# MattiaDallaCosta/JPEG-encoder-decoder

Measured on AMD Instinct MI355X. Metric: Mpixels/s encoded (device-resident BGR888 -> JFIF bytes), higher is better.
Workload: dtype int8-MFMA exact + fp64 replay (bit-exact); 1 GPU; config 3: 256 x 3840x2160 BGR888 frames per GPU, 4:2:0, Q=50, one independent JFIF per frame; frames_per_gpu=256, width=3840, height=2160, quality=50, mode=encode, pipeline=fused, parallelism=frame-parallel x1

## Files before the change

jpeg-encoder-decoder_amd/csrc/mij_kernels.hip:

```cpp
#include <stdlib.h>

#include "mij_internal.h"
#include "mij_headers.h"
#include "mij_colour_f64.h"

namespace mij {

typedef int v4i __attribute__((ext_vector_type(4)));
typedef unsigned u4v __attribute__((ext_vector_type(4)));
typedef unsigned short us2 __attribute__((ext_vector_type(2)));

__constant__ int c_zigzag[64] = {
    0,  1,  8,  16, 9,  2,  3,  10, 17, 24, 32, 25, 18, 11, 4,  5,
    12, 19, 26, 33, 40, 48, 41, 34, 27, 20, 13, 6,  7,  14, 21, 28,
    35, 42, 49, 56, 57, 50, 43, 36, 29, 22, 15, 23, 30, 37, 44, 51,
    58, 59, 52, 45, 38, 31, 39, 46, 53, 60, 61, 54, 47, 55, 62, 63};

#define SQRT1_2 0.70710678118654752440

__device__ __forceinline__ void wave_lds_sync() {
  __builtin_amdgcn_fence(__ATOMIC_RELEASE, "wavefront");
  __builtin_amdgcn_wave_barrier();
  __builtin_amdgcn_fence(__ATOMIC_ACQUIRE, "wavefront");
}

template <int N>
__device__ __forceinline__ uint32_t row_shr0(uint32_t x) {
  return (uint32_t)__builtin_amdgcn_update_dpp(0, (int)x, 0x110 + N, 0xF, 0xF, true);
}
__device__ __forceinline__ uint32_t row_scan16(uint32_t x) {
  x += row_shr0<1>(x);
  x += row_shr0<2>(x);
  x += row_shr0<4>(x);
  x += row_shr0<8>(x);
  return x;
}
__device__ __forceinline__ uint32_t row_last(uint32_t x) {
  return (uint32_t)__builtin_amdgcn_update_dpp(0, (int)x, 0x15F, 0xF, 0xF, false);
}
__device__ __forceinline__ uint32_t wave_scan64(uint32_t x) {
  x = row_scan16(x);
  x += (uint32_t)__builtin_amdgcn_update_dpp(0, (int)x, 0x142, 0xA, 0xF, false);
  x += (uint32_t)__builtin_amdgcn_update_dpp(0, (int)x, 0x143, 0xC, 0xF, false);
  return x;
}

__device__ __forceinline__ int mag_class(int v) {
  v = v < 0 ? -v : v;
  return 32 - __clz(v);
}

__device__ __forceinline__ uint32_t mag_bits(int v, int cls) {
  uint32_t id = (uint32_t)(v < 0 ? -v : v);
  if (v < 0) id = ~id;
  return id & ((1u << cls) - 1u);
}

// ... 34 lines not shown
  }
  if (ey) atomicOr(&lut[0 * LUT_WORDS + (i >> 5)], 1u << (i & 31));
  if (ecb) atomicOr(&lut[1 * LUT_WORDS + (i >> 5)], 1u << (i & 31));
  if (ecr) atomicOr(&lut[2 * LUT_WORDS + (i >> 5)], 1u << (i & 31));
}


__device__ __forceinline__ int dc_exact(int S, int q) {
  double f = __dmul_rn(__dmul_rn((double)S, SQRT1_2), SQRT1_2);
  f = __dmul_rn(f, 0.25);
  int t = (int)__ddiv_rn(f, (double)q);
  return t < -2048 ? -2048 : (t > 2047 ? 2047 : t);
}

__device__ __forceinline__ int dc_fast(int S, int q8, float inv8q, bool &tie) {
  const int s = S >> 31;
  const int a = (S ^ s) - s;
  const int k = (int)fmaf((float)a, inv8q, 2e-4f);
  tie = a != 0 && k * q8 == a;
  return (k ^ s) - s;
}

__device__ __forceinline__ int dc_tie(int d, const uint32_t *bits) {
  const int s = d >> 31;
  int k = (d ^ s) - s;
  k -= (int)((bits[k >> 5] >> (k & 31)) & 1u);
  return (k ^ s) - s;
}

struct TilePos {
  int f, tx, ty, valid_px;
};

__device__ __forceinline__ TilePos tile_pos(const Geom &G, int t) {
  TilePos p;
  p.f = (int)div_by((uint32_t)t, G.tpf_m, G.tpf_s);
  const int rem = t - p.f * G.tiles_per_frame;
  p.ty = (int)div_by((uint32_t)rem, G.tx_m, G.tx_s);
  p.tx = rem - p.ty * G.tiles_x;
  p.valid_px = min(TILE_W, G.w - p.tx * TILE_W);
  return p;
}

__device__ __forceinline__ TilePos tile_pos_r(const Geom &G, const int2 *fd, int t, bool &ok) {
  TilePos p = tile_pos(G, t);
  const FGeom fg = frame_geom(G, fd, p.f);
  p.valid_px = min(TILE_W, fg.w - p.tx * TILE_W);
  ok = p.tx < fg.tiles_x && p.ty < fg.rows;
  return p;
}

typedef __attribute__((address_space(3))) void lds_void_t;
typedef __attribute__((address_space(1))) void global_void_t;
constexpr int TILE_RAW = TILE_W * 3 * TILE_H;

constexpr int DMA_K = TILE_H / 2;
struct DmaOff {
  uint32_t v;
};
__device__ __forceinline__ DmaOff dma_offsets(int pitch, int lane) {
  const int l = lane < 48 ? lane : 0;
  return DmaOff{(uint32_t)((l / 24) * pitch + (l % 24) * 16)};
}
template <int K>
__device__ __forceinline__ void dma_one(uint32_t off, uint32_t lds, const uint8_t *src) {
  asm volatile("s_mov_b32 m0, %1\n\tglobal_load_lds_dwordx4 %0, %2 nt" : : "v"(off), "s"(lds), "s"(src)
               : "memory", "m0");
}
__device__ __forceinline__ void issue_tile_dma(const K1Args &a, const TilePos &p, int lane, uint8_t *raw,
                                               const DmaOff &off) {
  const uint64_t srcv = (uint64_t)(uintptr_t)(a.in + (long long)p.f * a.in_fs +
                                              (long long)(p.ty * TILE_H) * a.pitch + p.tx * TILE_W * 3);
  const uint32_t src_hi = (uint32_t)__builtin_amdgcn_readfirstlane((uint32_t)(srcv >> 32));
  const uint32_t src_lo = (uint32_t)__builtin_amdgcn_readfirstlane((uint32_t)srcv);
  const uint8_t *src = (const uint8_t *)(uintptr_t)(((uint64_t)src_hi << 32) | (uint64_t)src_lo);
  const uint32_t lds0 = __builtin_amdgcn_readfirstlane((uint32_t)(uintptr_t)(lds_void_t *)raw);
  const long long step = 2LL * a.pitch;
  const bool on = lane < 48 && (p.valid_px == TILE_W || (lane % 24) * 16 < p.valid_px * 3);
  if (on) {
    dma_one<0>(off.v, lds0, src);
    dma_one<1>(off.v, lds0 + 768, src + step);
    dma_one<2>(off.v, lds0 + 1536, src + 2 * step);
    dma_one<3>(off.v, lds0 + 2304, src + 3 * step);
    dma_one<4>(off.v, lds0 + 3072, src + 4 * step);
    dma_one<5>(off.v, lds0 + 3840, src + 5 * step);
    dma_one<6>(off.v, lds0 + 4608, src + 6 * step);
    dma_one<7>(off.v, lds0 + 5376, src + 7 * step);
  }
}
static_assert(DMA_K == 8 && TILE_W * 3 * 2 == 768, "issue_tile_dma: 8 instructions of 2 rows x 384 B");

__device__ __forceinline__ void dma_wait() { asm volatile("s_waitcnt vmcnt(0)" ::: "memory"); }
__device__ __forceinline__ void dma_wait_behind_stores() { asm volatile("s_waitcnt vmcnt(6)" ::: "memory"); }

template <int N>
__device__ __forceinline__ float ubyte_f32(uint32_t w) {
  float r;
  if constexpr (N == 0) asm("v_cvt_f32_ubyte0 %0, %1" : "=v"(r) : "v"(w));
  else if constexpr (N == 1) asm("v_cvt_f32_ubyte1 %0, %1" : "=v"(r) : "v"(w));
  else if constexpr (N == 2) asm("v_cvt_f32_ubyte2 %0, %1" : "=v"(r) : "v"(w));
  else asm("v_cvt_f32_ubyte3 %0, %1" : "=v"(r) : "v"(w));
  return r;
}

typedef float f2v __attribute__((ext_vector_type(2)));

__device__ __forceinline__ uint32_t pack_i16x2(int lo, int hi) {
  return __builtin_amdgcn_perm((uint32_t)hi, (uint32_t)lo, 0x05040100u);
}

__device__ __forceinline__ f2v pk_add_k(f2v a, float k) {
  f2v r;
  const unsigned long long kk = __float_as_uint(k);
  asm("v_pk_add_f32 %0, %1, %2 op_sel_hi:[1,0]" : "=v"(r) : "v"(a), "s"(kk));
  return r;
}

constexpr float CH_BIAS = 127.5f + 0x1p-16f;
constexpr float MAGIC = 12582912.0f;
constexpr uint32_t MAGIC_BITS = 0x4B400000u;
// ... 159 lines not shown
    for (int dy = 0; dy < 2; dy++)
      if (__ballot(r[dy].cy)) {
        const uint32_t corr = y_fix<RGB, GLOBAL_LUT>(w[it][dy][0], w[it][dy][1], w[it][dy][2], r[dy].yb, lut,
                                                     c4 | (pr << 5));
        if (corr) *Yd[dy] = py[dy] - corr;
      }
    if (__ballot(r[0].pd * r[1].pd == 0.0f)) {
      uint32_t cbc[2][4], crc[2][4];
#pragma unroll
      for (int dy = 0; dy < 2; dy++)
        chroma_fix<RGB, GLOBAL_LUT>(w[it][dy][0], w[it][dy][1], w[it][dy][2], lut, cbc[dy], crc[dy], c4 | (pr << 5));
      const uint32_t nb0 = cbc[0][0] + cbc[0][1] + cbc[1][0] + cbc[1][1];
      const uint32_t nb1 = cbc[0][2] + cbc[0][3] + cbc[1][2] + cbc[1][3];
      const uint32_t nr0 = crc[0][0] + crc[0][1] + crc[1][0] + crc[1][1];
      const uint32_t nr1 = crc[0][2] + crc[0][3] + crc[1][2] + crc[1][3];
      if (nb0 | nb1) *(uint16_t *)C0 = (uint16_t)chroma_pair(r[0].cbm, r[1].cbm, nb0, nb1);
      if (nr0 | nr1) *(uint16_t *)(C0 + 8 * LDS_BLK) = (uint16_t)chroma_pair(r[0].crm, r[1].crm, nr0, nr1);
    }
  }
}

constexpr uint32_t TOK_AC = 1u << 10;
constexpr uint32_t LB_NOTOK = TOK_AC | 0xFFu;
constexpr uint32_t SEG_DC_ONLY = 1u << 31;

__device__ __forceinline__ uint32_t &tok_at(uint32_t *base, uint32_t i) {
  return *(uint32_t *)((char *)base + (i << 2));
}
__device__ __forceinline__ void emit_tokens(const int (&o)[16], int lane, int g, int bcol,
                                            bool valid, bool chroma, bool dc_diffed,
                                            bool first_pred, int pred0,
                                            uint32_t *segtok, uint32_t segoff, uint32_t *tok0, uint32_t *segcnt, uint32_t *hDC,
                                            uint32_t *hAC, int16_t (*st)[16], int kflags = 0, bool acz = false, bool dc_only = false) {
  if (acz && dc_only) {
    const int dc0 = o[0];
    const int prev = (int)row_shr0<1>((uint32_t)dc0);
    const unsigned long long vb = __ballot(valid && g == 0);
    if (g == 0) {
      if ((bcol & 7) == 7) *segcnt = SEG_DC_ONLY | (uint32_t)__popcll(vb);
      if (valid && (bcol & 7) != 0) atomicAdd(&hDC[mag_class(dc0 - prev)], 1u);
    }
    if (lane == 0 && vb) atomicAdd(&hAC[0x00], (unsigned)__popcll(vb));
    return;
  }
  uint32_t Mlo = 0, Mhi = 0;
  const int zsw = 8 * (bcol & 7);
  if (!acz) {
  u4v c0, c1;
#pragma unroll
  for (int k = 0; k < 4; k++) {
    c0[k] = pack_i16x2(o[2 * k], o[2 * k + 1]);
    c1[k] = pack_i16x2(o[8 + 2 * k], o[9 + 2 * k]);
  }
  int16_t *stb = &st[0][0] + 64 * bcol;
  *(u4v *)(stb + ((16 * g) ^ zsw)) = c0;
  *(u4v *)(stb + ((16 * g + 8) ^ zsw)) = c1;
  uint32_t pm;
  asm("v_pk_min_u16 %0, %1, 1 op_sel_hi:[1,0]" : "=v"(pm) : "v"(c0[0]));
#pragma unroll
  for (int k = 1; k < 8; k++) {
    const uint32_t w = k < 4 ? c0[k] : c1[k - 4];
    uint32_t h;
    asm("v_pk_min_u16 %0, %1, 1 op_sel_hi:[1,0]" : "=v"(h) : "v"(w));
    asm("v_lshl_or_b32 %0, %1, %2, %3" : "=v"(pm) : "v"(h), "i"(2 * k), "v"(pm));
  }
  uint32_t m16 = (pm & 0x5555u) | ((pm >> 15) & 0xAAAAu);
  if (g == 0) m16 &= ~1u;
  uint32_t h = m16 << (16 * (g & 1));
  const auto r16 = __builtin_amdgcn_permlane16_swap(h, h, false, false);
  h = r16[0] | r16[1];
  const auto r32 = __builtin_amdgcn_permlane32_swap(h, h, false, false);
  Mlo = r32[0];
  Mhi = r32[1];
  }
  const int eob = !(Mhi >> 31);
  const int n = valid ? 1 + __popc(Mlo) + __popc(Mhi) + eob : 0;
  const int pos = chroma ? (bcol & 7) : bcol;
  uint32_t incl = row_scan16((uint32_t)n);
  if (chroma)
    incl -= (uint32_t)__builtin_amdgcn_update_dpp(0, (int)incl, 0x157, 0xF, 0xF, false) & (0u - (uint32_t)(bcol >> 3));
  const int base = (int)incl - n;
  const int dc0 = o[0];
  const int prev = (int)row_shr0<1>((uint32_t)dc0);
  wave_lds_sync();
  if (pos == (chroma ? 7 : 15)) {
    if (g == 0) *segcnt = incl;
    if ((uint32_t)g < ((0u - incl) & 3u)) tok_at(segtok, segoff + incl + (uint32_t)g) = LB_NOTOK;
  }
  if (g == 0) {
    if (valid) {
      if (dc_diffed || pos != 0 || first_pred) {
        const int diff = dc_diffed ? dc0 : dc0 - (pos != 0 ? prev : pred0);
        const int cls = mag_class(diff);
        const uint32_t tk = (uint32_t)cls | (mag_bits(diff, cls) << 16);
        if (pos == 0) *tok0 = tk;
        else tok_at(segtok, segoff + base) = tk;
        atomicAdd(&hDC[cls], 1u);
      }
      if (eob) tok_at(segtok, segoff + base + n - 1) = TOK_AC;
    }
  }
  {
    const unsigned long long eobs = __ballot(g == 0 && valid && eob);
    if (lane == 0 && eobs) atomicAdd(&hAC[0x00], (unsigned)__popcll(eobs));
  }
  if (!acz && valid && !(kflags & K1F_NO_ACLOOP)) {
    const int16_t *sl = &st[0][0] + 64 * bcol;
    auto token = [&](int z, int rank, int zp) {
      const int cz = sl[z ^ zsw];
      const int m = cz + (cz >> 31);
      uint32_t lead;
      asm("v_ffbh_i32 %0, %1" : "=v"(lead) : "v"(m));
      const uint32_t cls = 32u - lead;
      const uint32_t mag = __builtin_amdgcn_ubfe((uint32_t)m, 0u, cls);
      const uint32_t runp = (uint32_t)(z + zp);
      const uint32_t t = (runp << 4) + cls;
      if (!(kflags & K1F_NO_TOKSTORE)) tok_at(segtok, segoff + (uint32_t)(base + rank)) = t | (mag << 16);
      if (!(kflags & K1F_NO_HIST)) {
        atomicAdd(&hAC[t & 255u], 1u);
        if (runp >= 80u) atomicAdd(&hAC[0xF0], (runp - 64u) >> 4);
      }
    };
    const uint32_t cm = 0x11111111u << g;
    const int rank_lo = __popc(Mlo), zp_lo = 31 - __clz((int)(Mlo | 1u));
    const uint32_t M1 = Mlo | 1u;
    for (uint32_t m = Mlo & cm; m; m &= m - 1u) {
      const int z = __builtin_ctz(m);
      const uint32_t bef = __builtin_amdgcn_ubfe(M1, 0u, (uint32_t)z);
      uint32_t lz;
      asm("v_ffbh_u32 %0, %1" : "=v"(lz) : "v"(bef));
      token(z, __popc(bef), 32 + (int)lz);
    }
    const int rank_lo1 = rank_lo + 1;
    for (uint32_t m = Mhi & cm; m; m &= m - 1u) {
      const int zz = __builtin_ctz(m);
      const uint32_t bef = __builtin_amdgcn_ubfe(Mhi, 0u, (uint32_t)zz);
      uint32_t lz;
      asm("v_ffbh_u32 %0, %1" : "=v"(lz) : "v"(bef));
      token(32 + zz, rank_lo1 + __popc(bef), (int)min(lz, (uint32_t)(63 - zp_lo)));
    }
  }
  wave_lds_sync();
}

constexpr int K1M_COEF_OUT = 1;
constexpr int K1M_TOK_OUT = 2;
constexpr int K1M_COEF_IN = 4;
constexpr int K1M_RGB = 8;
constexpr int K1M_REGIONS = 16;
constexpr int K1M_AUDIT = 32;
constexpr int K1M_FLOOR = 64;
constexpr int k1_base(int mode) { return mode & ~(K1M_RGB | K1M_REGIONS | K1M_AUDIT | K1M_FLOOR); }

template <int MODE>
constexpr bool k1_wide() { return k1_base(MODE) == K1M_COEF_OUT || k1_base(MODE) == K1M_TOK_OUT; }
template <int MODE>
constexpr int k1_waves() {
  return k1_wide<MODE>() ? 12 : 4;
}

template <int MODE>
__global__ __launch_bounds__(64 * k1_waves<MODE>(), k1_wide<MODE>() ? 1 : 2) void k_mcu_dct(K1Args a) {
  constexpr bool PIX = !(MODE & K1M_COEF_IN);
  constexpr bool TOK = MODE & K1M_TOK_OUT;
  constexpr int NW = k1_waves<MODE>();
  constexpr int NT = 64 * NW;
  constexpr bool DEFER = k1_base(MODE) == K1M_COEF_OUT;
  constexpr bool RGB = MODE & K1M_RGB;
  constexpr bool REG = MODE & K1M_REGIONS;
  constexpr bool AUDIT = MODE & K1M_AUDIT;
  constexpr bool FLOOR = MODE & K1M_FLOOR;
  const int2 *const fdims = REG ? a.fdims : nullptr;
  __shared__ __attribute__((aligned(16))) uint8_t s_raw[PIX ? NW : 1][TILE_RAW];
  __shared__ __attribute__((aligned(16))) uint8_t s_tile[PIX ? NW : 1][LDS_WAVE];
  __shared__ __attribute__((aligned(16))) int4 s_A[PIX ? 12 * 64 : 1];
  __shared__ __attribute__((aligned(16))) float s_fac[2][64];
  __shared__ float s_inv8q[2];
  __shared__ uint32_t s_dctie[2][DCTIE_WORDS];
  constexpr bool LUT_LDS = PIX && !(TOK && NW >= 8);
  __shared__ uint32_t s_lut[LUT_LDS ? 3 * LUT_WORDS : 1];
  __shared__ double s_cos[64];
  __shared__ uint8_t s_zz[64];
  __shared__ int s_qint[2][64];
  __shared__ __attribute__((aligned(16))) int s_czl[PIX ? 64 : 1];
  __shared__ __attribute__((aligned(16))) int16_t s_st[TOK ? NW : 1][64][16];
  constexpr int HREP = PIX ? 1 : 4;
  __shared__ uint32_t s_hac[TOK ? 2 : 1][2][HREP][256];
  __shared__ uint32_t s_hdc[TOK ? 2 : 1][2][HREP][16];
  __shared__ int s_next;

  const Tables *__restrict__ T = a.tab;
#ifdef MIJ_K1_DIAG
  const int kflags = a.flags;
#else
  constexpr int kflags = 0;
#endif
  if (threadIdx.x < 64) {
    s_cos[threadIdx.x] = T->cosd[threadIdx.x];
    s_zz[threadIdx.x] = (uint8_t)c_zigzag[threadIdx.x];
  }
  if (TOK) {
    for (int i = threadIdx.x; i < 2 * 2 * HREP * 256; i += NT) (&s_hac[0][0][0][0])[i] = 0;
    for (int i = threadIdx.x; i < 2 * 2 * HREP * 16; i += NT) (&s_hdc[0][0][0][0])[i] = 0;
  }
  if (threadIdx.x < 128) s_qint[threadIdx.x >> 6][threadIdx.x & 63] = T->qint[threadIdx.x >> 6][threadIdx.x & 63];
  if (threadIdx.x < 2) s_inv8q[threadIdx.x] = 1.0f / (float)(8 * T->qint[threadIdx.x][0]);
  if (PIX && threadIdx.x < 64) s_czl[threadIdx.x] = T->czl[threadIdx.x];
  if (threadIdx.x < 2 * DCTIE_WORDS) (&s_dctie[0][0])[threadIdx.x] = (&T->dctie[0][0])[threadIdx.x];
  if (PIX) {
    for (int i = threadIdx.x; i < 12 * 64; i += NT) s_A[i] = T->mfma_a[i];
    if (LUT_LDS)
      for (int i = threadIdx.x; i < 3 * LUT_WORDS; i += NT) s_lut[i] = (&T->lut[0][0])[i];
  }
  const uint32_t *__restrict__ lut = LUT_LDS ? (const uint32_t *)s_lut : &T->lut[0][0];
  for (int i = threadIdx.x; i < 128; i += NT) {
    s_fac[i >> 6][i & 63] = T->qfac[i >> 6][i & 63];
  }
  if (threadIdx.x == 0) s_next = (int)blockIdx.x * a.per_wg + NW;
  if (blockIdx.x == 0)
    for (int i = threadIdx.x; i < a.nerr_zero; i += NT) a.err_zero[i] = 0;
  __syncthreads();

  const int lane = threadIdx.x & 63;
  const int wave = __builtin_amdgcn_readfirstlane(threadIdx.x >> 6);
  uint8_t *L = s_tile[PIX ? wave : 0];
  const int g = lane >> 4, bcol = lane & 15;
  const int c4 = lane & 31, pr = lane >> 5;
  const uint32_t kq = (uint32_t)T->kq[g];
  const int q_dc[2] = {T->qint[0][0], T->qint[1][0]};
  const bool cz_on = PIX && !AUDIT && T->cz_on;
  const Geom &G = a.g;
  const int bw = G.w >> 3, mw = G.w >> 4;
  const int ntiles = a.nframes * G.tiles_per_frame;
  const int t0 = (int)blockIdx.x * a.per_wg;
  const int f0 = t0 / G.tiles_per_frame;
  const int tend = min(ntiles, t0 + a.per_wg);
  int t = t0 + wave;
  auto skip_outside = [&](int &tt) {
    bool ok;
    while (tt < tend && (tile_pos_r(G, fdims, tt, ok), !ok)) {
      int v = 0;
      if (lane == 0) v = atomicAdd(&s_next, 1);
      tt = __builtin_amdgcn_readfirstlane(v);
    }
  };
  auto tpos = [&](int tt) {
    bool ok;
    return REG ? tile_pos_r(G, fdims, tt, ok) : tile_pos(G, tt);
  };
  if (REG) skip_outside(t);
#ifdef MIJ_K1_DIAG
  const unsigned long long w_t0 = __builtin_amdgcn_s_memrealtime();
  int w_ntiles = 0;
  unsigned long long ph[5] = {0, 0, 0, 0, 0}, tph = __builtin_amdgcn_s_memtime();
#define K1_PHASE(k)                                                  \
  do {                                                               \
    const unsigned long long tn_ = __builtin_amdgcn_s_memtime();     \
    ph[k] += tn_ - tph;                                              \
    tph = tn_;                                                       \
  } while (0)
#else
#define K1_PHASE(k)
#endif
  uint32_t nrep = 0;
  if (t < tend) {
    uint8_t *raw = s_raw[PIX ? wave : 0];
    TilePos p = tpos(t);
    const DmaOff doff = dma_offsets(a.pitch, lane);
    if (PIX) issue_tile_dma(a, p, lane, raw, doff);
    auto load_coefs = [&](const TilePos &pp, u4v (&dst)[PIX ? 1 : 3][2]) {
#pragma unroll
      for (int nt = 0; nt < 3; nt++) {
        bool valid;
        long long blk;
        const FGeom fg = frame_geom(G, fdims, pp.f);
        const int bwf = REG ? fg.bw : bw, mwf = REG ? fg.mw : mw;
        const int nYf = REG ? fg.nY : G.nY, nCf = REG ? fg.nC : G.nC;
        if (nt < 2) {
          const int bx = pp.tx * 16 + bcol;
          valid = bx < bwf;
          blk = (long long)(2 * pp.ty + nt) * bwf + bx;
        } else {
          const int mx = pp.tx * 8 + (bcol & 7);
          valid = mx < mwf;
          blk = nYf + (bcol >= 8 ? nCf : 0) + (long long)pp.ty * mwf + mx;
        }
        dst[PIX ? 0 : nt][0] = dst[PIX ? 0 : nt][1] = u4v{0, 0, 0, 0};
        if (valid) {
          const int16_t *src = a.coef + (long long)pp.f * G.coef_fs + blk * 64 + 16 * g;
          dst[PIX ? 0 : nt][0] = *(const u4v *)src;
          dst[PIX ? 0 : nt][1] = *(const u4v *)(src + 8);
        }
      }
    };
    u4v cnext[PIX ? 1 : 3][2];
    if (!PIX) load_coefs(p, cnext);
    bool first = true;
    for (;;) {
      TilePos pn = p;
      int tn = 0;
      if (lane == 0) tn = atomicAdd(&s_next, 1);
      tn = __builtin_amdgcn_readfirstlane(tn);
      uint32_t fl_w = 0;
      if (PIX) {
        K1_PHASE(3);
        if (first || (kflags & (K1F_NO_DCT | K1F_NO_STORE)))
          dma_wait();
        else if (DEFER)
          dma_wait_behind_stores();
        K1_PHASE(0);
        if (!(kflags & K1F_NO_COLOUR) && !FLOOR) colour_stage<RGB, !LUT_LDS>(raw, L, c4, pr, lut, !(kflags & K1F_NO_LUT));
        if (FLOOR) fl_w = ((const uint32_t *)raw)[lane];
        wave_lds_sync();
        K1_PHASE(1);
        if (REG) skip_outside(tn);
        if (tn < tend) {
          pn = tpos(tn);
          issue_tile_dma(a, pn, lane, raw, doff);
        }
        K1_PHASE(2);
      } else {
        if (REG) skip_outside(tn);
        if (tn < tend) pn = tpos(tn);
      }

      const bool do_dct = !(kflags & K1F_NO_DCT);
      auto dct_digit = [&](const int d, v4i (&acc)[4], const v4i Bf) {
#pragma unroll
        for (int m = 0; m < 4; m++) {
          const int4 F = s_A[(3 * m + d) * 64 + lane];
#ifdef MIJ_K1_DIAG
          if (kflags & K1F_EXTRA_LDS) {
            v4i dummy;
            asm volatile("ds_read_b128 %0, %1\n\ts_waitcnt lgkmcnt(0)" : "=v"(dummy) : "v"((uint32_t)(uintptr_t)(lds_void_t *)&s_A[(3 * m + d) * 64 + lane]) : "memory");
          }
#endif
          const v4i Fv = {F.x, F.y, F.z, F.w};
          v4i c;
          if (d == 0) {
            c = v4i{1 << 17, 0, 1 << 17, 0};
          } else {
            typedef unsigned long long u64x2 __attribute__((ext_vector_type(2)));
            c = __builtin_bit_cast(v4i, __builtin_bit_cast(u64x2, acc[m]) << 7);
          }
          acc[m] = (kflags & K1F_NO_MFMA) ? c + Fv + Bf
                                          : __builtin_amdgcn_mfma_i32_16x16x64_i8(Fv, Bf, c, 0, 0, 0);
        }
        if (d == 2) {
#pragma unroll
          for (int m = 0; m < 4; m++) {
            acc[m][0] ^= (int)0x80000000u;
            acc[m][2] ^= (int)0x80000000u;
          }
        }
      };
      auto dct_ntile = [&](const int nt, v4i (&acc)[4], uint32_t &lc) {
        const v4i Bp = *(const v4i *)(L + (nt * 16 + bcol) * LDS_BLK + 16 * g);
        uint32_t l1 = 0;
#pragma unroll
        for (int k = 0; k < 4; k++) l1 = __builtin_amdgcn_sad_u8((uint32_t)Bp[k], 0x80808080u, l1);
        const auto r16 = __builtin_amdgcn_permlane16_swap(l1, l1, false, false);
        l1 = r16[0] + r16[1];
        const auto r32 = __builtin_amdgcn_permlane32_swap(l1, l1, false, false);
        const uint32_t L1 = r32[0] + r32[1];
        if (nt < 2) {
          lc = (L1 >> 1) + 1u;
        } else {
          lc = __float_as_uint(fmaf((float)L1, 0.72f, 80.0f));
        }
        const v4i Bf = Bp ^ (int)0x80808080;
#pragma unroll
        for (int d = 0; d < 3; d++) dct_digit(d, acc, Bf);
      };

      u4v pre[PIX ? 1 : 3][2];
// ... 41 lines not shown
#pragma unroll
          for (int k = 0; k < 4; k++) {
            s0[k] = pack_i16x2(o[2 * k], o[2 * k + 1]);
            s1[k] = pack_i16x2(o[8 + 2 * k], o[9 + 2 * k]);
          }
          int16_t *const fcoef = a.coef + (long long)p.f * G.coef_fs;
          if (kflags & (K1F_LINEAR_STORE | K1F_PLAIN_STORE)) {
            int16_t *dst = fcoef + (long long)blk * 64 + 16 * g;
            if (!valid) {
            } else if (kflags & K1F_LINEAR_STORE) {
              const long long b0 = nt < 2 ? blk - bcol : G.nY + (long long)p.ty * mw + p.tx * 8;
              int16_t *lin = fcoef + b0 * 64 + 8 * lane;
              __builtin_nontemporal_store(s0, (u4v *)lin);
              __builtin_nontemporal_store(s1, (u4v *)(lin + 512));
            } else {
              *(u4v *)dst = s0;
              *(u4v *)(dst + 8) = s1;
            }
          } else {
            u4v d1, d2;
#pragma unroll
            for (int k = 0; k < 4; k++) {
              d1[k] = (uint32_t)__builtin_amdgcn_update_dpp((int)s0[k], (int)s1[k], 0x128, 0xF, 0xC, false);
              d2[k] = (uint32_t)__builtin_amdgcn_update_dpp((int)s1[k], (int)s0[k], 0x128, 0xF, 0x3, false);
            }
            const int off = 16 * g + 8 * (bcol >> 3);
            int b1, b2;
            const bool v1 = block_at(nt, bcol & 7, b1), v2 = block_at(nt, bcol | 8, b2);
            int16_t *const p1 = fcoef + (long long)b1 * 64 + off;
            if (v1) __builtin_nontemporal_store(d1, (u4v *)p1);
            if (v1 || v2) __builtin_nontemporal_store(v2 ? d2 : d1, (u4v *)(v2 ? fcoef + (long long)b2 * 64 + off : p1));
          }
        }
        if (PIX && valid && g == 0) a.dc[(long long)p.f * G.nblk + blk] = (int16_t)o[0];
        if (TOK && !(kflags & K1F_NO_EMIT)) {
          const long long fs = (long long)p.f * G.nseg + seg;
          const int slot = p.f - f0;
          int pred0 = 0;
          const bool first_pred = !PIX && a.seg_dc_inline;
          if (first_pred && valid && g == 0 && (comp == 1 ? (bcol & 7) : bcol) == 0) {
            const FGeom fg = frame_geom(G, fdims, p.f);
            const int nYf = REG ? fg.nY : G.nY, nCf = REG ? fg.nC : G.nC;
            const int cstart = comp == 0 ? 0 : (bcol >= 8 ? nYf + nCf : nYf);
            pred0 = blk == cstart ? (a.dc_pred ? (int)a.dc_pred[p.f * 4 + (comp == 0 ? 0 : (bcol >= 8 ? 2 : 1))] : 0)
                                  : (int)a.dc[(long long)p.f * G.nblk + blk - 1];
          }
          emit_tokens(o, lane, g, bcol, valid, comp == 1, !PIX && a.dc_diffed, first_pred, pred0,
                      a.tok + (long long)p.f * G.nseg * SEG_TOK, (uint32_t)seg * SEG_TOK, a.tok0 + fs,
                      a.seg_ntok + fs, s_hdc[TOK ? slot : 0][comp][bcol & (HREP - 1)],
                      s_hac[TOK ? slot : 0][comp][bcol & (HREP - 1)],
                      s_st[TOK ? wave : 0], kflags, acz, PIX && !REG && a.dc_only);
        }
      };
      if (FLOOR) {
#pragma unroll
        for (int nt = 0; nt < 3; nt++) {
          int o[16];
#pragma unroll
          for (int k = 0; k < 16; k++) o[k] = (int)(fl_w >> k) & 0xFF;
          finish(nt, o, false);
        }
      } else if (PIX && do_dct) {
        constexpr bool PIPE = TOK;
        v4i accs[PIPE ? 2 : 1][4];
        uint32_t lcs[PIPE ? 2 : 1];
        if (PIPE) dct_ntile(0, accs[0], lcs[0]);
#pragma unroll
        for (int nt = 0; nt < 3; nt++) {
          const int comp = nt == 2 ? 1 : 0;
          const int cur = PIPE ? (nt & 1) : 0;
          if (!PIPE) {
            dct_ntile(nt, accs[0], lcs[0]);
          } else if (nt + 1 < 3) {
            dct_ntile(nt + 1, accs[PIPE ? (cur ^ 1) : 0], lcs[PIPE ? (cur ^ 1) : 0]);
          }
          v4i(&acc)[4] = accs[cur];
          const uint32_t lcb = lcs[cur];
          int o[16];
          if constexpr (!AUDIT) {
            if (nt == 2 && cz_on) {
              const int4 *czl = (const int4 *)&s_czl[16 * g];
              uint32_t all = ~0u;
#pragma unroll
              for (int m = 0; m < 4; m++) {
                const int4 Lq = czl[m];
                const int Lv[4] = {Lq.x, Lq.y, Lq.z, Lq.w};
#pragma unroll
                for (int r = 0; r < 4; r++) {
                  const uint32_t lo = (uint32_t)acc[m][r] - (uint32_t)Lv[r], hi = (uint32_t)acc[m][r] + (uint32_t)Lv[r];
                  all &= lo & ~hi;
                }
              }
              bool fails = (int)all >= 0;
              if constexpr (TOK) {
                uint32_t ccol;
                asm volatile("v_and_b32 %0, 7, %1" : "=v"(ccol) : "v"(lane));
                fails = fails && (int)ccol < (p.valid_px >> 4);
              }
              if (!__ballot(fails)) {
#pragma unroll
                for (int k = 0; k < 16; k++) o[k] = 0;
                bool tie;
                const int dcv = dc_fast(acc[0][0], 8 * q_dc[comp], s_inv8q[comp], tie);
                if (g == 0) o[0] = dcv;
                if (__ballot(tie && g == 0))
                  if (g == 0 && tie) o[0] = dc_tie(dcv, s_dctie[comp]);
                K1_PHASE(3);
                finish(nt, o, true);
                K1_PHASE(4);
                continue;
              }
            }
          }
          uint32_t hz;
          uint32_t xq[4] = {0u, 0u, 0u, 0u};
          auto lquant = [&](int n, uint32_t E1, uint32_t EE, uint32_t kq, uint32_t &x) -> int {
            const int sgn = n >> 31;
            uint32_t hi;
            asm("v_xad_u32 %0, %1, %2, %3" : "=v"(hi) : "v"(n), "v"(sgn), "v"(E1));
            uint32_t lo;
            asm("v_sub_u32_e64 %0, %1, %2 clamp" : "=v"(lo) : "v"(hi), "v"(EE));
            x = __builtin_amdgcn_bitop3_b32(x, hi, lo, 0xF6);
            return (n >> kq) - sgn;
          };
          if (kflags & K1F_NO_QUANT) {
#pragma unroll
            for (int k = 0; k < 16; k++) o[k] = acc[k >> 2][k & 3];
            hz = 0;
          } else if (nt < 2) {
            const uint32_t E = lcb;
            const uint32_t E1 = E + 1u, EE = 2u * E + 1u;
#pragma unroll
            for (int k = 0; k < 16; k++) o[k] = lquant(acc[k >> 2][k & 3], E1, EE, kq, xq[k >> 2]);
            hz = (xq[0] | xq[1] | xq[2] | xq[3]) >> kq;
          } else {
            int slo = 0, shi = 0;
#pragma unroll
            for (int m = 0; m < 4; m++) {
              const float4 fac = *(const float4 *)&s_fac[comp][16 * g + 4 * m];
// ... 32 lines not shown
                const int k = 4 * m + r;
                if (nt < 2) {
                  const uint32_t E = lcb;
                  uint32_t x = 0;
                  (void)lquant(acc[m][r], E + 1u, 2u * E + 1u, kq, x);
                  mm |= (uint32_t)((x >> kq) != 0) << k;
                } else {
                  const float nf = (float)acc[m][r];
                  const float fa = s_fac[comp][16 * g + k];
                  const float tv = fmaf(fa, __uint_as_float(lcb), 1.0e-6f);
                  mm |= (uint32_t)((int)fmaf(nf, fa, -tv) != (int)fmaf(nf, fa, tv)) << k;
                }
              }
            }
            return mm;
          };
          auto need_mtiles = [&]() -> uint32_t {
            if (nt < 2) {
              uint32_t nd = 0;
#pragma unroll
              for (int m = 0; m < 4; m++) nd |= (uint32_t)((xq[m] >> kq) != 0u) << m;
              return nd;
            }
            const uint32_t d01 = xq[0] != xq[1], d23 = (xq[2] - xq[0]) != (xq[3] - xq[1]);
            return d01 * 3u + d23 * 12u;
          };
          if constexpr (AUDIT) {
            int blk;
            if (block_of(nt, blk)) a.audit[((long long)p.f * G.nblk + blk) * 4 + g] = (uint16_t)straddle_mask(0xFu);
          }
          {
            bool tie;
            const int dcv = dc_fast(acc[0][0], 8 * q_dc[comp], s_inv8q[comp], tie);
            if (g == 0) o[0] = dcv;
            if (__ballot(tie && g == 0))
              if (g == 0 && tie) o[0] = dc_tie(dcv, s_dctie[comp]);
          }
          if constexpr (DEFER) {
            const unsigned long long need = __ballot(hz != 0);
            if (need && !(kflags & K1F_NO_REPLAY)) {
              int blk;
              const bool valid = block_of(nt, blk);
              const unsigned long long vm = __ballot(valid);
              const uint32_t m16 = (uint32_t)((need | need >> 16 | need >> 32 | need >> 48) & vm) & 0xFFFFu;
              if (m16 && lane == 0) {
                a.fix_mask[(long long)t * 3 + nt] = (uint16_t)m16;
                nrep += (uint32_t)__popc(m16);
              }
            }
          }
          if (!DEFER && __ballot(hz != 0) && !(kflags & K1F_NO_REPLAY)) {
            const uint32_t mm = straddle_mask(need_mtiles());
            if (!(kflags & K1F_COUNT_LUMA) || nt < 2)
              nrep += (kflags & K1F_COUNT_PASSES) ? (uint32_t)(lane == 0) : (uint32_t)__popc(mm);
            if constexpr (TOK) {
              const int c = __popc(mm);
              const int incl = (int)wave_scan64((uint32_t)c);
              const int T = __builtin_amdgcn_readlane(incl, 63);
              const int base = incl - c;
              uint16_t *lst = (uint16_t *)&s_st[wave][0][0];
              int *res = (int *)((uint8_t *)&s_st[wave][0][0] + 256);
              for (int c0 = 0; c0 < T; c0 += 64) {
                {
                  uint32_t m2 = mm;
                  for (int idx = base; m2; idx++) {
                    const int k = __ffs(m2) - 1;
                    m2 &= m2 - 1u;
                    if (idx >= c0 && idx < c0 + 64) lst[idx - c0] = (uint16_t)(lane << 4 | k);
                  }
                }
                wave_lds_sync();
                const int nch = min(T - c0, 64);
                for (int r = 0; r < nch && !(kflags & K1F_REPLAY_NO_FP64); r += 8) {
                  const int j = r + (lane >> 3), x = lane & 7;
                  const int e = lst[j < nch ? j : 0];
                  const int ol = e >> 4, k = e & 15;
                  const int z = 16 * (ol >> 4) + k;
                  const int rz = s_zz[z], v = rz >> 3, u = rz & 7;
                  const uint8_t *Pb = L + (nt * 16 + (ol & 15)) * LDS_BLK;
                  double in = 0.0;
#pragma unroll
                  for (int y = 0; y < 8; y++)
                    in = __dadd_rn(in, __dmul_rn((double)((int)Pb[y * 8 + x] - 128), s_cos[y * 8 + v]));
                  double freq = 0.0;
#pragma unroll
                  for (int xx = 0; xx < 8; xx++)
                    freq = __dadd_rn(freq, __dmul_rn(__shfl(in, (lane & ~7) + xx), s_cos[xx * 8 + u]));
                  if (u == 0) freq = __dmul_rn(freq, SQRT1_2);
                  if (v == 0) freq = __dmul_rn(freq, SQRT1_2);
                  freq = __dmul_rn(freq, 0.25);
                  int tq = (int)__ddiv_rn(freq, (double)s_qint[comp][z]);
                  tq = tq < -2048 ? -2048 : (tq > 2047 ? 2047 : tq);
                  if (x == 0 && j < nch) res[j] = tq;
                }
                wave_lds_sync();
                {
                  uint32_t m2 = mm;
                  for (int idx = base; m2; idx++) {
                    const int k = __ffs(m2) - 1;
                    m2 &= m2 - 1u;
                    if (idx >= c0 && idx < c0 + 64) {
                      const int v = res[idx - c0];
#pragma unroll
                      for (int jj = 0; jj < 16; jj++) o[jj] = jj == k ? v : o[jj];
                    }
                  }
                }
                wave_lds_sync();
              }
            }
          }
          if (nt == 0 && !DEFER && !(kflags & K1F_NO_DMAWAIT)) dma_wait();
          K1_PHASE(3);
          finish(nt, o, false);
          K1_PHASE(4);
        }
      } else if (!PIX) {
#pragma unroll
        for (int nt = 0; nt < 3; nt++) {
          int o[16];
          finish(nt, o, false);
        }
      }
      if (PIX) wave_lds_sync();
#ifdef MIJ_K1_DIAG
      w_ntiles++;
#endif
      if (tn >= tend) break;
      p = pn;
      t = tn;
      first = false;
    }
  }
  if (__ballot(nrep != 0)) {
    const uint32_t tot = wave_scan64(nrep);
    if (lane == 63) atomicAdd(a.replays, tot);
  }
#ifdef MIJ_K1_DIAG
  if (a.wtime && lane == 0) {
    unsigned long long *w = a.wtime + K1_WTIME_WORDS * ((long long)blockIdx.x * NW + wave);
    w[0] = w_t0;
    w[1] = __builtin_amdgcn_s_memrealtime();
    w[2] = (unsigned long long)w_ntiles;
    for (int k = 0; k < 5; k++) w[3 + k] = ph[k];
  }
#endif
  if (TOK) {
    __syncthreads();
    for (int i = threadIdx.x; i < 2 * 2 * 256; i += NT) {
      const int slot = i >> 9, tb = (i >> 8) & 1, sym = i & 255;
      uint32_t v = 0;
#pragma unroll
      for (int c = 0; c < HREP; c++) v += s_hac[slot][tb][c][sym];
      if (v && f0 + slot < a.nframes)
        atomicAdd(&a.hist[((long long)(f0 + slot) * 4 + (tb ? 3 : 1)) * 257 + sym], v);
    }
    if (threadIdx.x < 64) {
      const int slot = threadIdx.x >> 5, tb = (threadIdx.x >> 4) & 1, sym = threadIdx.x & 15;
      uint32_t v = 0;
#pragma unroll
      for (int c = 0; c < HREP; c++) v += s_hdc[slot][tb][c][sym];
      if (v && f0 + slot < a.nframes)
        atomicAdd(&a.hist[((long long)(f0 + slot) * 4 + (tb ? 2 : 0)) * 257 + sym], v);
    }
  }
}


__device__ __forceinline__ int y_ref(const uint8_t *px, int ib, int ir) { return y_f64(px[ir], px[1], px[ib]); }
__device__ __forceinline__ int cb_ref(const uint8_t *px, int ib, int ir) { return cb_f64(px[ir], px[1], px[ib]); }
__device__ __forceinline__ int cr_ref(const uint8_t *px, int ib, int ir) { return cr_f64(px[ir], px[1], px[ib]); }

__global__ __launch_bounds__(256) void k_fix_blocks(K1Args a) {
  __shared__ __attribute__((aligned(8))) uint8_t s_px[4][64];
  __shared__ double s_inner[4][64];
  __shared__ double s_cos[64];
  __shared__ int s_q[2][64];
  const Tables *__restrict__ T = a.tab;
  if (threadIdx.x < 64) s_cos[threadIdx.x] = T->cosd[threadIdx.x];
  if (threadIdx.x < 128) s_q[threadIdx.x >> 6][threadIdx.x & 63] = T->qint[threadIdx.x >> 6][threadIdx.x & 63];
  __syncthreads();
  const int lane = threadIdx.x & 63, wave = threadIdx.x >> 6;
  const Geom G = a.g;
  const int x = lane & 7, y = lane >> 3;
  const int rz = c_zigzag[lane], v = rz >> 3, u = rz & 7;
  const int ib = a.rgb ? 2 : 0, ir = 2 - ib;
  const long long nmask = (long long)a.nframes * G.tiles_per_frame * 3;
  for (long long base = ((long long)blockIdx.x * 4 + wave) * 64; base < nmask; base += (long long)gridDim.x * 4 * 64) {
    const long long e = base + lane;
    const uint32_t mk = e < nmask ? a.fix_mask[e] : 0u;
    unsigned long long any = __ballot(mk != 0);
    if (mk) a.fix_mask[e] = 0;
    while (any) {
      const int l = __ffsll((long long)any) - 1;
      any &= any - 1ull;
      uint32_t mm = (uint32_t)__builtin_amdgcn_readlane((int)mk, l);
      const int tg = (int)((base + l) / 3), nt = (int)(base + l - 3LL * tg);
      const int f = tg / G.tiles_per_frame, rem = tg - f * G.tiles_per_frame;
      const int ty = rem / G.tiles_x, tx = rem - ty * G.tiles_x;
// ... 2530 lines not shown
```

Before: 611,500 Mpixels/s.

## Cap token K1 VGPRs and rematerialize kernel args to cut register pressure

Moves the K1 body into a device function and specializes the wide token kernels with an explicit VGPR cap. To fit under that cap, it reloads tile addressing arguments from the kernarg segment via scalar loads, replaces lane-id comparisons with inverse-ballot mask predicates (SGPR rather than VGPR), folds uniform flags into one SGPR, and reuses a single LDS buffer for the replay list and its results. It also moves the first DMA wait out of the loop and simplifies the valid-column test. The VGPR cap can cause spills, and the reload adds scalar memory latency on every tile.

```diff
diff --git a/jpeg-encoder-decoder_amd/csrc/mij_kernels.hip b/jpeg-encoder-decoder_amd/csrc/mij_kernels.hip
--- a/jpeg-encoder-decoder_amd/csrc/mij_kernels.hip
+++ b/jpeg-encoder-decoder_amd/csrc/mij_kernels.hip
@@ -23,6 +23,8 @@
   __builtin_amdgcn_wave_barrier();
   __builtin_amdgcn_fence(__ATOMIC_ACQUIRE, "wavefront");
 }
+
+__device__ __forceinline__ bool lane_in(unsigned long long mask) { return __builtin_amdgcn_inverse_ballot_w64(mask); }
 
 template <int N>
 __device__ __forceinline__ uint32_t row_shr0(uint32_t x) {
@@ -123,14 +125,43 @@
   int f, tx, ty, valid_px;
 };
 
+struct TileArgs {
+  const uint8_t *in;
+  long long in_fs;
+  uint32_t tpf_m, tpf_s, tx_m, tx_s;
+};
+typedef const __attribute__((address_space(4))) K1Args *k1_kernarg_t;
+__device__ __forceinline__ TileArgs tile_args(const K1Args &a) {
+  return TileArgs{a.in, a.in_fs, a.g.tpf_m, a.g.tpf_s, a.g.tx_m, a.g.tx_s};
+}
+static_assert(offsetof(K1Args, in_fs) == offsetof(K1Args, in) + 8 && offsetof(Geom, tx_s) == offsetof(Geom, tpf_m) + 12,
+              "tile_args_reload: two 16-byte loads");
+__device__ __forceinline__ TileArgs tile_args_reload(k1_kernarg_t ka) {
+  u4v src, mag;
+  asm volatile("s_load_dwordx4 %0, %2, %3\n\ts_load_dwordx4 %1, %2, %4\n\ts_waitcnt lgkmcnt(0)"
+               : "=&s"(src), "=&s"(mag)
+               : "s"(ka), "i"(offsetof(K1Args, in)), "i"(offsetof(K1Args, g) + offsetof(Geom, tpf_m)));
+  TileArgs r;
+  r.in = (const uint8_t *)(uintptr_t)((uint64_t)src[0] | (uint64_t)src[1] << 32);
+  r.in_fs = (long long)((uint64_t)src[2] | (uint64_t)src[3] << 32);
+  r.tpf_m = mag[0];
+  r.tpf_s = mag[1];
+  r.tx_m = mag[2];
+  r.tx_s = mag[3];
+  return r;
+}
+
+__device__ __forceinline__ TilePos tile_pos(const Geom &G, const TileArgs &ta, int t) {
+  TilePos p;
+  p.f = (int)div_by((uint32_t)t, ta.tpf_m, ta.tpf_s);
+  const int rem = t - p.f * G.tiles_per_frame;
+  p.ty = (int)div_by((uint32_t)rem, ta.tx_m, ta.tx_s);
+  p.tx = rem - p.ty * G.tiles_x;
+  p.valid_px = min(TILE_W / 8, (G.w >> 3) - p.tx * (TILE_W / 8)) * 8;
+  return p;
+}
 __device__ __forceinline__ TilePos tile_pos(const Geom &G, int t) {
-  TilePos p;
-  p.f = (int)div_by((uint32_t)t, G.tpf_m, G.tpf_s);
-  const int rem = t - p.f * G.tiles_per_frame;
-  p.ty = (int)div_by((uint32_t)rem, G.tx_m, G.tx_s);
-  p.tx = rem - p.ty * G.tiles_x;
-  p.valid_px = min(TILE_W, G.w - p.tx * TILE_W);
-  return p;
+  return tile_pos(G, TileArgs{nullptr, 0, G.tpf_m, G.tpf_s, G.tx_m, G.tx_s}, t);
 }
 
 __device__ __forceinline__ TilePos tile_pos_r(const Geom &G, const int2 *fd, int t, bool &ok) {
@@ -148,35 +179,36 @@
 constexpr int DMA_K = TILE_H / 2;
 struct DmaOff {
   uint32_t v;
+  int col;
 };
 __device__ __forceinline__ DmaOff dma_offsets(int pitch, int lane) {
   const int l = lane < 48 ? lane : 0;
-  return DmaOff{(uint32_t)((l / 24) * pitch + (l % 24) * 16)};
+  return DmaOff{(uint32_t)((l / 24) * pitch + (l % 24) * 16), lane < 48 ? (lane % 24) * 16 : 0x7FFFFFFF};
 }
 template <int K>
 __device__ __forceinline__ void dma_one(uint32_t off, uint32_t lds, const uint8_t *src) {
   asm volatile("s_mov_b32 m0, %1\n\tglobal_load_lds_dwordx4 %0, %2 nt" : : "v"(off), "s"(lds), "s"(src)
                : "memory", "m0");
 }
-__device__ __forceinline__ void issue_tile_dma(const K1Args &a, const TilePos &p, int lane, uint8_t *raw,
+__device__ __forceinline__ void issue_tile_dma(const TileArgs &ta, const TilePos &p, uint32_t lds_raw, int step2,
                                                const DmaOff &off) {
-  const uint64_t srcv = (uint64_t)(uintptr_t)(a.in + (long long)p.f * a.in_fs +
-                                              (long long)(p.ty * TILE_H) * a.pitch + p.tx * TILE_W * 3);
+  const uint32_t lds0 = (uint32_t)__builtin_amdgcn_readfirstlane(lds_raw);
+  const long long step = __builtin_amdgcn_readfirstlane(step2);
+  const uint64_t srcv = (uint64_t)(uintptr_t)(ta.in + (long long)p.f * ta.in_fs +
+                                              (long long)(p.ty * (TILE_H / 2)) * step + p.tx * TILE_W * 3);
   const uint32_t src_hi = (uint32_t)__builtin_amdgcn_readfirstlane((uint32_t)(srcv >> 32));
   const uint32_t src_lo = (uint32_t)__builtin_amdgcn_readfirstlane((uint32_t)srcv);
   const uint8_t *src = (const uint8_t *)(uintptr_t)(((uint64_t)src_hi << 32) | (uint64_t)src_lo);
-  const uint32_t lds0 = __builtin_amdgcn_readfirstlane((uint32_t)(uintptr_t)(lds_void_t *)raw);
-  const long long step = 2LL * a.pitch;
-  const bool on = lane < 48 && (p.valid_px == TILE_W || (lane % 24) * 16 < p.valid_px * 3);
+  const bool on = off.col < p.valid_px * 3;
   if (on) {
     dma_one<0>(off.v, lds0, src);
     dma_one<1>(off.v, lds0 + 768, src + step);
-    dma_one<2>(off.v, lds0 + 1536, src + 2 * step);
-    dma_one<3>(off.v, lds0 + 2304, src + 3 * step);
-    dma_one<4>(off.v, lds0 + 3072, src + 4 * step);
-    dma_one<5>(off.v, lds0 + 3840, src + 5 * step);
-    dma_one<6>(off.v, lds0 + 4608, src + 6 * step);
-    dma_one<7>(off.v, lds0 + 5376, src + 7 * step);
+    dma_one<2>(off.v, lds0 + 1536, src + 2 * (long long)step);
+    dma_one<3>(off.v, lds0 + 2304, src + 3 * (long long)step);
+    dma_one<4>(off.v, lds0 + 3072, src + 4 * (long long)step);
+    dma_one<5>(off.v, lds0 + 3840, src + 5 * (long long)step);
+    dma_one<6>(off.v, lds0 + 4608, src + 6 * (long long)step);
+    dma_one<7>(off.v, lds0 + 5376, src + 7 * (long long)step);
   }
 }
 static_assert(DMA_K == 8 && TILE_W * 3 * 2 == 768, "issue_tile_dma: 8 instructions of 2 rows x 384 B");
@@ -402,15 +434,18 @@
                                             bool first_pred, int pred0,
                                             uint32_t *segtok, uint32_t segoff, uint32_t *tok0, uint32_t *segcnt, uint32_t *hDC,
                                             uint32_t *hAC, int16_t (*st)[16], int kflags = 0, bool acz = false, bool dc_only = false) {
+  const bool g0 = lane_in(0xFFFFull);
+  const bool seg_last = lane_in(chroma ? 0x8080808080808080ull : 0x8000800080008000ull);
+  const bool seg_rest = lane_in(chroma ? 0xFEFEull : 0xFFFEull);
   if (acz && dc_only) {
     const int dc0 = o[0];
     const int prev = (int)row_shr0<1>((uint32_t)dc0);
-    const unsigned long long vb = __ballot(valid && g == 0);
-    if (g == 0) {
-      if ((bcol & 7) == 7) *segcnt = SEG_DC_ONLY | (uint32_t)__popcll(vb);
-      if (valid && (bcol & 7) != 0) atomicAdd(&hDC[mag_class(dc0 - prev)], 1u);
-    }
-    if (lane == 0 && vb) atomicAdd(&hAC[0x00], (unsigned)__popcll(vb));
+    const unsigned long long vb = __ballot(valid && g0);
+    if (g0) {
+      if (seg_last) *segcnt = SEG_DC_ONLY | (uint32_t)__popcll(vb);
+      if (valid && seg_rest) atomicAdd(&hDC[mag_class(dc0 - prev)], 1u);
+    }
+    if (vb && lane_in(1ull)) atomicAdd(&hAC[0x00], (unsigned)__popcll(vb));
     return;
   }
   uint32_t Mlo = 0, Mhi = 0;
@@ -435,7 +470,7 @@
     asm("v_lshl_or_b32 %0, %1, %2, %3" : "=v"(pm) : "v"(h), "i"(2 * k), "v"(pm));
   }
   uint32_t m16 = (pm & 0x5555u) | ((pm >> 15) & 0xAAAAu);
-  if (g == 0) m16 &= ~1u;
+  if (g0) m16 &= ~1u;
   uint32_t h = m16 << (16 * (g & 1));
   const auto r16 = __builtin_amdgcn_permlane16_swap(h, h, false, false);
   h = r16[0] | r16[1];
@@ -445,7 +480,6 @@
   }
   const int eob = !(Mhi >> 31);
   const int n = valid ? 1 + __popc(Mlo) + __popc(Mhi) + eob : 0;
-  const int pos = chroma ? (bcol & 7) : bcol;
   uint32_t incl = row_scan16((uint32_t)n);
   if (chroma)
     incl -= (uint32_t)__builtin_amdgcn_update_dpp(0, (int)incl, 0x157, 0xF, 0xF, false) & (0u - (uint32_t)(bcol >> 3));
@@ -453,26 +487,26 @@
   const int dc0 = o[0];
   const int prev = (int)row_shr0<1>((uint32_t)dc0);
   wave_lds_sync();
-  if (pos == (chroma ? 7 : 15)) {
-    if (g == 0) *segcnt = incl;
+  if (seg_last) {
+    if (g0) *segcnt = incl;
     if ((uint32_t)g < ((0u - incl) & 3u)) tok_at(segtok, segoff + incl + (uint32_t)g) = LB_NOTOK;
   }
-  if (g == 0) {
+  if (g0) {
     if (valid) {
-      if (dc_diffed || pos != 0 || first_pred) {
-        const int diff = dc_diffed ? dc0 : dc0 - (pos != 0 ? prev : pred0);
+      if (dc_diffed || seg_rest || first_pred) {
+        const int diff = dc_diffed ? dc0 : dc0 - (seg_rest ? prev : pred0);
         const int cls = mag_class(diff);
         const uint32_t tk = (uint32_t)cls | (mag_bits(diff, cls) << 16);
-        if (pos == 0) *tok0 = tk;
-        else tok_at(segtok, segoff + base) = tk;
+        if (seg_rest) tok_at(segtok, segoff + base) = tk;
+        else *tok0 = tk;
         atomicAdd(&hDC[cls], 1u);
       }
       if (eob) tok_at(segtok, segoff + base + n - 1) = TOK_AC;
     }
   }
   {
-    const unsigned long long eobs = __ballot(g == 0 && valid && eob);
-    if (lane == 0 && eobs) atomicAdd(&hAC[0x00], (unsigned)__popcll(eobs));
+    const unsigned long long eobs = __ballot(g0 && valid && eob);
+    if (eobs && lane_in(1ull)) atomicAdd(&hAC[0x00], (unsigned)__popcll(eobs));
   }
   if (!acz && valid && !(kflags & K1F_NO_ACLOOP)) {
     const int16_t *sl = &st[0][0] + 64 * bcol;
@@ -530,7 +564,7 @@
 }
 
 template <int MODE>
-__global__ __launch_bounds__(64 * k1_waves<MODE>(), k1_wide<MODE>() ? 1 : 2) void k_mcu_dct(K1Args a) {
+__device__ __forceinline__ void k1_body(const K1Args &a) {
   constexpr bool PIX = !(MODE & K1M_COEF_IN);
   constexpr bool TOK = MODE & K1M_TOK_OUT;
   constexpr int NW = k1_waves<MODE>();
@@ -595,10 +629,12 @@
   const int wave = __builtin_amdgcn_readfirstlane(threadIdx.x >> 6);
   uint8_t *L = s_tile[PIX ? wave : 0];
   const int g = lane >> 4, bcol = lane & 15;
+  const bool g0 = lane_in(0xFFFFull), l0 = lane_in(1ull);
   const int c4 = lane & 31, pr = lane >> 5;
   const uint32_t kq = (uint32_t)T->kq[g];
   const int q_dc[2] = {T->qint[0][0], T->qint[1][0]};
-  const bool cz_on = PIX && !AUDIT && T->cz_on;
+  const int uflags0 = __builtin_amdgcn_readfirstlane(((PIX && !AUDIT && T->cz_on) ? 1 : 0) |
+                                                     ((PIX && !REG && a.dc_only) ? 2 : 0));
   const Geom &G = a.g;
   const int bw = G.w >> 3, mw = G.w >> 4;
   const int ntiles = a.nframes * G.tiles_per_frame;
@@ -610,13 +646,16 @@
     bool ok;
     while (tt < tend && (tile_pos_r(G, fdims, tt, ok), !ok)) {
       int v = 0;
-      if (lane == 0) v = atomicAdd(&s_next, 1);
+      if (l0) v = atomicAdd(&s_next, 1);
       tt = __builtin_amdgcn_readfirstlane(v);
     }
   };
-  auto tpos = [&](int tt) {
+  constexpr bool RELOAD = PIX && !REG && TOK;
+  const k1_kernarg_t ka = (k1_kernarg_t)__builtin_amdgcn_kernarg_segment_ptr();
+  auto targs = [&]() { return RELOAD ? tile_args_reload(ka) : tile_args(a); };
+  auto tpos = [&](int tt, const TileArgs &ta) {
     bool ok;
-    return REG ? tile_pos_r(G, fdims, tt, ok) : tile_pos(G, tt);
+    return REG ? tile_pos_r(G, fdims, tt, ok) : tile_pos(G, ta, tt);
   };
   if (REG) skip_outside(t);
 #ifdef MIJ_K1_DIAG
@@ -635,9 +674,12 @@
   uint32_t nrep = 0;
   if (t < tend) {
     uint8_t *raw = s_raw[PIX ? wave : 0];
-    TilePos p = tpos(t);
+    const TileArgs ta0 = targs();
+    TilePos p = tpos(t, ta0);
     const DmaOff doff = dma_offsets(a.pitch, lane);
-    if (PIX) issue_tile_dma(a, p, lane, raw, doff);
+    const uint32_t raw_lds = (uint32_t)(uintptr_t)(lds_void_t *)&s_raw[0][0] + (uint32_t)(PIX ? wave : 0) * TILE_RAW;
+    const int dma_step = 2 * a.pitch;
+    if (PIX) issue_tile_dma(ta0, p, raw_lds, dma_step, doff);
     auto load_coefs = [&](const TilePos &pp, u4v (&dst)[PIX ? 1 : 3][2]) {
 #pragma unroll
       for (int nt = 0; nt < 3; nt++) {
@@ -665,16 +707,19 @@
     };
     u4v cnext[PIX ? 1 : 3][2];
     if (!PIX) load_coefs(p, cnext);
-    bool first = true;
+    if (PIX) dma_wait();
     for (;;) {
       TilePos pn = p;
+      int uflags = uflags0;
+      if constexpr (!REG) asm volatile("" : "+s"(uflags));
+      const bool cz_on = PIX && !AUDIT && (uflags & 1), dc_only = PIX && !REG && (uflags & 2);
       int tn = 0;
-      if (lane == 0) tn = atomicAdd(&s_next, 1);
+      if (l0) tn = atomicAdd(&s_next, 1);
       tn = __builtin_amdgcn_readfirstlane(tn);
       uint32_t fl_w = 0;
       if (PIX) {
         K1_PHASE(3);
-        if (first || (kflags & (K1F_NO_DCT | K1F_NO_STORE)))
+        if (kflags & (K1F_NO_DCT | K1F_NO_STORE))
           dma_wait();
         else if (DEFER)
           dma_wait_behind_stores();
@@ -685,13 +730,14 @@
         K1_PHASE(1);
         if (REG) skip_outside(tn);
         if (tn < tend) {
-          pn = tpos(tn);
-          issue_tile_dma(a, pn, lane, raw, doff);
+          const TileArgs ta = targs();
+          pn = tpos(tn, ta);
+          issue_tile_dma(ta, pn, raw_lds, dma_step, doff);
         }
         K1_PHASE(2);
       } else {
         if (REG) skip_outside(tn);
-        if (tn < tend) pn = tpos(tn);
+        if (tn < tend) pn = tpos(tn, targs());
       }
 
       const bool do_dct = !(kflags & K1F_NO_DCT);
@@ -707,10 +753,10 @@
 #endif
           const v4i Fv = {F.x, F.y, F.z, F.w};
           v4i c;
+          typedef unsigned long long u64x2 __attribute__((ext_vector_type(2)));
           if (d == 0) {
-            c = v4i{1 << 17, 0, 1 << 17, 0};
+            c = __builtin_bit_cast(v4i, u64x2{1ull << 17, 1ull << 17});
           } else {
-            typedef unsigned long long u64x2 __attribute__((ext_vector_type(2)));
             c = __builtin_bit_cast(v4i, __builtin_bit_cast(u64x2, acc[m]) << 7);
           }
           acc[m] = (kflags & K1F_NO_MFMA) ? c + Fv + Bf
@@ -818,13 +864,13 @@
             if (v1 || v2) __builtin_nontemporal_store(v2 ? d2 : d1, (u4v *)(v2 ? fcoef + (long long)b2 * 64 + off : p1));
           }
         }
-        if (PIX && valid && g == 0) a.dc[(long long)p.f * G.nblk + blk] = (int16_t)o[0];
+        if (PIX && valid && g0) a.dc[(long long)p.f * G.nblk + blk] = (int16_t)o[0];
         if (TOK && !(kflags & K1F_NO_EMIT)) {
           const long long fs = (long long)p.f * G.nseg + seg;
           const int slot = p.f - f0;
           int pred0 = 0;
           const bool first_pred = !PIX && a.seg_dc_inline;
-          if (first_pred && valid && g == 0 && (comp == 1 ? (bcol & 7) : bcol) == 0) {
+          if (first_pred && valid && g0 && (comp == 1 ? (bcol & 7) : bcol) == 0) {
             const FGeom fg = frame_geom(G, fdims, p.f);
             const int nYf = REG ? fg.nY : G.nY, nCf = REG ? fg.nC : G.nC;
             const int cstart = comp == 0 ? 0 : (bcol >= 8 ? nYf + nCf : nYf);
@@ -835,7 +881,7 @@
                       a.tok + (long long)p.f * G.nseg * SEG_TOK, (uint32_t)seg * SEG_TOK, a.tok0 + fs,
                       a.seg_ntok + fs, s_hdc[TOK ? slot : 0][comp][bcol & (HREP - 1)],
                       s_hac[TOK ? slot : 0][comp][bcol & (HREP - 1)],
-                      s_st[TOK ? wave : 0], kflags, acz, PIX && !REG && a.dc_only);
+                      s_st[TOK ? wave : 0], kflags, acz, dc_only);
         }
       };
       if (FLOOR) {
@@ -888,9 +934,9 @@
                 for (int k = 0; k < 16; k++) o[k] = 0;
                 bool tie;
                 const int dcv = dc_fast(acc[0][0], 8 * q_dc[comp], s_inv8q[comp], tie);
-                if (g == 0) o[0] = dcv;
-                if (__ballot(tie && g == 0))
-                  if (g == 0 && tie) o[0] = dc_tie(dcv, s_dctie[comp]);
+                if (g0) o[0] = dcv;
+                if (__ballot(tie && g0))
+                  if (g0 && tie) o[0] = dc_tie(dcv, s_dctie[comp]);
                 K1_PHASE(3);
                 finish(nt, o, true);
                 K1_PHASE(4);
@@ -989,9 +1035,9 @@
           {
             bool tie;
             const int dcv = dc_fast(acc[0][0], 8 * q_dc[comp], s_inv8q[comp], tie);
-            if (g == 0) o[0] = dcv;
-            if (__ballot(tie && g == 0))
-              if (g == 0 && tie) o[0] = dc_tie(dcv, s_dctie[comp]);
+            if (g0) o[0] = dcv;
+            if (__ballot(tie && g0))
+              if (g0 && tie) o[0] = dc_tie(dcv, s_dctie[comp]);
           }
           if constexpr (DEFER) {
             const unsigned long long need = __ballot(hz != 0);
@@ -1000,7 +1046,7 @@
               const bool valid = block_of(nt, blk);
               const unsigned long long vm = __ballot(valid);
               const uint32_t m16 = (uint32_t)((need | need >> 16 | need >> 32 | need >> 48) & vm) & 0xFFFFu;
-              if (m16 && lane == 0) {
+              if (m16 && l0) {
                 a.fix_mask[(long long)t * 3 + nt] = (uint16_t)m16;
                 nrep += (uint32_t)__popc(m16);
               }
@@ -1009,28 +1055,27 @@
           if (!DEFER && __ballot(hz != 0) && !(kflags & K1F_NO_REPLAY)) {
             const uint32_t mm = straddle_mask(need_mtiles());
             if (!(kflags & K1F_COUNT_LUMA) || nt < 2)
-              nrep += (kflags & K1F_COUNT_PASSES) ? (uint32_t)(lane == 0) : (uint32_t)__popc(mm);
+              nrep += (kflags & K1F_COUNT_PASSES) ? (uint32_t)(l0) : (uint32_t)__popc(mm);
             if constexpr (TOK) {
               const int c = __popc(mm);
               const int incl = (int)wave_scan64((uint32_t)c);
               const int T = __builtin_amdgcn_readlane(incl, 63);
               const int base = incl - c;
-              uint16_t *lst = (uint16_t *)&s_st[wave][0][0];
-              int *res = (int *)((uint8_t *)&s_st[wave][0][0] + 256);
+              int *lst = (int *)&s_st[wave][0][0];
               for (int c0 = 0; c0 < T; c0 += 64) {
                 {
                   uint32_t m2 = mm;
                   for (int idx = base; m2; idx++) {
                     const int k = __ffs(m2) - 1;
                     m2 &= m2 - 1u;
-                    if (idx >= c0 && idx < c0 + 64) lst[idx - c0] = (uint16_t)(lane << 4 | k);
+                    if (idx >= c0 && idx < c0 + 64) lst[idx - c0] = lane << 4 | k;
                   }
                 }
                 wave_lds_sync();
                 const int nch = min(T - c0, 64);
                 for (int r = 0; r < nch && !(kflags & K1F_REPLAY_NO_FP64); r += 8) {
                   const int j = r + (lane >> 3), x = lane & 7;
-                  const int e = lst[j < nch ? j : 0];
+                  const int e = lst[j < nch ? j : 0] & 0x3FF;
                   const int ol = e >> 4, k = e & 15;
                   const int z = 16 * (ol >> 4) + k;
                   const int rz = s_zz[z], v = rz >> 3, u = rz & 7;
@@ -1048,7 +1093,7 @@
                   freq = __dmul_rn(freq, 0.25);
                   int tq = (int)__ddiv_rn(freq, (double)s_qint[comp][z]);
                   tq = tq < -2048 ? -2048 : (tq > 2047 ? 2047 : tq);
-                  if (x == 0 && j < nch) res[j] = tq;
+                  if (x == 0 && j < nch) lst[j] = tq;
                 }
                 wave_lds_sync();
                 {
@@ -1057,7 +1102,7 @@
                     const int k = __ffs(m2) - 1;
                     m2 &= m2 - 1u;
                     if (idx >= c0 && idx < c0 + 64) {
-                      const int v = res[idx - c0];
+                      const int v = lst[idx - c0];
 #pragma unroll
                       for (int jj = 0; jj < 16; jj++) o[jj] = jj == k ? v : o[jj];
                     }
@@ -1086,15 +1131,14 @@
       if (tn >= tend) break;
       p = pn;
       t = tn;
-      first = false;
     }
   }
   if (__ballot(nrep != 0)) {
     const uint32_t tot = wave_scan64(nrep);
-    if (lane == 63) atomicAdd(a.replays, tot);
+    if (lane == 63) atomicAdd(ka->replays, tot);
   }
 #ifdef MIJ_K1_DIAG
-  if (a.wtime && lane == 0) {
+  if (a.wtime && l0) {
     unsigned long long *w = a.wtime + K1_WTIME_WORDS * ((long long)blockIdx.x * NW + wave);
     w[0] = w_t0;
     w[1] = __builtin_amdgcn_s_memrealtime();
@@ -1104,24 +1148,43 @@
 #endif
   if (TOK) {
     __syncthreads();
-    for (int i = threadIdx.x; i < 2 * 2 * 256; i += NT) {
+    int tid = threadIdx.x;
+    asm volatile("" : "+v"(tid));
+    uint32_t *const hist = ka->hist;
+    const int nf_left = ka->nframes - f0;
+    for (int i = tid; i < 2 * 2 * 256; i += NT) {
       const int slot = i >> 9, tb = (i >> 8) & 1, sym = i & 255;
       uint32_t v = 0;
 #pragma unroll
       for (int c = 0; c < HREP; c++) v += s_hac[slot][tb][c][sym];
-      if (v && f0 + slot < a.nframes)
-        atomicAdd(&a.hist[((long long)(f0 + slot) * 4 + (tb ? 3 : 1)) * 257 + sym], v);
-    }
-    if (threadIdx.x < 64) {
-      const int slot = threadIdx.x >> 5, tb = (threadIdx.x >> 4) & 1, sym = threadIdx.x & 15;
+      if (v && slot < nf_left)
+        atomicAdd(&hist[((long long)(f0 + slot) * 4 + (tb ? 3 : 1)) * 257 + sym], v);
+    }
+    if (tid < 64) {
+      const int slot = tid >> 5, tb = (tid >> 4) & 1, sym = tid & 15;
       uint32_t v = 0;
 #pragma unroll
       for (int c = 0; c < HREP; c++) v += s_hdc[slot][tb][c][sym];
-      if (v && f0 + slot < a.nframes)
-        atomicAdd(&a.hist[((long long)(f0 + slot) * 4 + (tb ? 2 : 0)) * 257 + sym], v);
-    }
-  }
-}
+      if (v && slot < nf_left)
+        atomicAdd(&hist[((long long)(f0 + slot) * 4 + (tb ? 2 : 0)) * 257 + sym], v);
+    }
+  }
+}
+
+template <int MODE>
+__global__ __launch_bounds__(64 * k1_waves<MODE>(), k1_wide<MODE>() ? 1 : 2) void k_mcu_dct(K1Args a) {
+  k1_body<MODE>(a);
+}
+#define K1_TOKEN_KERNEL(MODE)                                                                         \
+  template <>                                                                                         \
+  __global__ __launch_bounds__(64 * 12, 1) __attribute__((amdgpu_num_vgpr(83))) void k_mcu_dct<MODE>( \
+      K1Args a) {                                                                                     \
+    static_assert(k1_waves<MODE>() == 12 && k1_wide<MODE>(), "the wide token K1");                    \
+    k1_body<MODE>(a);                                                                                 \
+  }
+K1_TOKEN_KERNEL(K1M_TOK_OUT)
+K1_TOKEN_KERNEL(K1M_TOK_OUT | K1M_RGB)
+#undef K1_TOKEN_KERNEL
 
 
 __device__ __forceinline__ int y_ref(const uint8_t *px, int ib, int ir) { return y_f64(px[ir], px[1], px[ib]); }
```

Result: faster. 620,100 Mpixels/s (median of 6 runs) (+1.4%).
